# FordyceLab/magnify

Measured on AMD Instinct MI355X. Metric: megapixels/sec through flatfield+segment+ROI-reduce; markers/sec, higher is better.
Workload: dtype u16

## Files before the change

include/magnify_hip.h:

```cpp
#ifndef MAGNIFY_HIP_H
#define MAGNIFY_HIP_H

#include <stddef.h>
#include <stdint.h>

#ifdef __cplusplus
extern "C" {
#endif

#define MG_OK 0
#define MG_EINVAL (-1)
#define MG_ELAUNCH (-2)
#define MG_EIO (-3)

#define MG_U8 0
#define MG_U16 1
#define MG_F32 2
#define MG_F64 3

#define MG_NO_EDGE 100.0f
#define MG_SCORE_SKIPPED (-2.0f)

#define MG_WALK_MAX_Y 65535
#define MG_ZERO_WALK 1024
// ... 74 lines not shown
#define MG_PLANE_MINMAX_WALK 1024
int mg_plane_minmax(const void* d_src, int dtype, int n_planes, int64_t plane_stride, int h, int w,
                    int64_t row_stride, double* d_minmax, void* stream);


#define MG_ROTATE_WALK 2048
int mg_affine_bilinear(const void* d_src, void* d_dst, int dtype, int64_t n_planes, int h, int w,
                       const double* matrix, const double* offset, double* d_minmax, void* stream);

int64_t mg_shading_workspace_bytes(int n, int w);
int64_t mg_shading_offset(int n, int w, int field);
int mg_shading_downsample(const void* d_tiles, int dtype, int64_t n, int ty, int tx, int w, float* d_out, void* stream);
int mg_shading_prepare(void* d_ws, int n, int w, void* stream);
int mg_shading_dct2(void* d_ws, int n, int w, const double* d_in, double* d_out, int inverse, void* stream);
int mg_shading_alm_begin(void* d_ws, int n, int w, int get_darkfield, int max_iterations, double mu, double lam_f,
                         double lam_d, double tol, double norm_f, double b_up, void* stream);
int mg_shading_alm_iterate(void* d_ws, int n, int w, int k, int get_darkfield, void* stream);
int mg_shading_reweight(void* d_ws, int n, int w, double epsilon, void* stream);
int mg_shading_upsample(const double* d_flat_w, const double* d_dark_w, int w, int ty, int tx, double* d_partial,
                        float* d_flat, float* d_dark, void* stream);
#define MG_SHADING_APPLY_WALK 2048
#define MG_SHADING_SETUP_WALK 1024
int mg_shading_apply_stitch(const void* d_tiles, int dtype, int n_fields, int64_t planes_per_field, int n_tile_rows,
                            int n_tile_cols, int ty, int tx, int overlap, const float* d_flat, const float* d_dark,
                            void* d_image, double* d_minmax, void* stream);
int mg_shading_apply_stitch_blend(const void* d_tiles, int dtype, int n_fields, int64_t planes_per_field,
                                  int n_tile_rows, int n_tile_cols, int ty, int tx, int overlap, const float* d_flat,
                                  const float* d_dark, void* d_image, double* d_minmax, void* stream);

int mg_shading_apply_stitch_shift(const void* d_tiles, int dtype, int n_fields, int64_t planes_per_field,
                                  int n_tile_rows, int n_tile_cols, int ty, int tx, int overlap, const float* d_flat,
                                  const float* d_dark, void* d_image, double* d_minmax, const int32_t* d_shift,
                                  int n_tables, int n_time, int blend, void* stream);


int mg_to_uint8_blur(const void* d_src, int dtype, int n_planes, int64_t plane_stride, int h, int w,
                     int64_t row_stride, const double* d_minmax, uint8_t* d_blur, uint8_t* d_u8, void* stream);

int mg_scharr_hist(const uint8_t* d_blur, int n_planes, int h, int w, int mode, const uint32_t* d_base,
                   uint32_t* d_hist, uint32_t* d_scratch, int64_t scratch_words, void* stream);
int64_t mg_scharr_hist_scratch_words(int n_planes, int h, int w, int mode);

int mg_to_uint8_blur_hist(const void* d_src, int dtype, int n_planes, int64_t plane_stride, int h, int w,
                          int64_t row_stride, const double* d_minmax, uint8_t* d_blur, uint8_t* d_u8, uint32_t* d_hist,
                          uint32_t* d_scratch, int64_t scratch_words, void* stream);
int64_t mg_blur_hist_scratch_words(int n_planes, int h, int w);

int mg_edge_thresholds(const uint32_t* d_hist, int n_planes, const int64_t* ranks4, float gamma_low, float gamma_high,
                       int32_t* d_thresh, float* d_quantiles, int32_t* d_unresolved, int32_t* d_state,
                       uint32_t* d_win_base, void* stream);
int mg_edge_thresholds_window(const uint32_t* d_hist_win, int n_planes, int pass, float gamma_low, float gamma_high,
                              int32_t* d_state, uint32_t* d_win_base, int32_t* d_thresh, float* d_quantiles,
                              int32_t* d_unresolved, void* stream);


int mg_canny_nms(const uint8_t* d_blur, int n_planes, int h, int w, const int32_t* d_thresh, uint32_t* d_weak,
                 uint32_t* d_strong, uint32_t* d_class, int64_t words_per_plane, void* stream);
int mg_canny_nms_strips(int w, int* strip_w, int* wave_rows, int* group_rows);

int mg_canny_hysteresis(const uint32_t* d_weak, uint32_t* d_strong, int64_t words_per_plane, int n_planes, int h,
                        int w, uint32_t* d_changed, const uint8_t* d_flags_in, uint8_t* d_flags_out, void* stream);
int mg_hysteresis_tiles(int h, int w, int* tiles_x, int* tiles_y);

#define MG_UNPACK_BITS_WALK 4096
int mg_unpack_bits(const uint32_t* d_bits, int64_t words_per_plane, int n_planes, int64_t n_bits, uint8_t* d_out,
                   void* stream);

int64_t mg_edge_grid_scan_words(int n_planes, int h, int w, int grid);
int mg_edge_grid(const uint32_t* d_edge_bits, int64_t words_per_plane, int n_planes, int h, int w, int grid,
                 int32_t* d_cell_counts, int32_t* d_cell_starts, int32_t* d_num_edges, int32_t* d_coords,
                 int64_t coord_cap, uint64_t* d_scan_state, int32_t* d_edge_totals, int phases, void* stream);

#define MG_EDGE_ANGLES_WALK 1048576
int mg_edge_angles(const uint8_t* d_blur, int n_planes, int h, int w, const int32_t* d_coords, int64_t coord_cap,
                   const int32_t* d_num_edges, float* d_angle, void* stream);


int mg_dedup_layout(int h, int w, int min_r, int max_r, int* n_tile_rows, int* n_tile_cols, int64_t* n_layers,
                    int64_t* bitmap_words);

#define MG_CANDIDATES_WALK 2048
#define MG_CANDIDATES_TAB_WALK 1024
#define MG_CANDIDATES_TAB_FILL 1024
int mg_candidate_circles(const int32_t* d_coords, int64_t coord_cap, const int32_t* d_cell_starts,
                         const int32_t* d_cell_counts, const int32_t* d_num_edges, int n_planes, int h, int w,
                         int grid, const uint64_t* d_seeds, int64_t num_iter, int min_r, int max_r,
                         uint32_t* d_bitmap, int64_t bitmap_words, float* d_raw, void* stream);

int mg_candidate_keys(const int32_t* d_coords, int64_t coord_cap, const int32_t* d_cell_starts,
                      const int32_t* d_cell_counts, const int32_t* d_num_edges, int n_planes, int h, int w, int grid,
                      const uint64_t* d_seeds, int64_t num_iter, int min_r, int max_r, uint32_t* d_keys, float* d_raw,
                      void* stream);

int mg_keys_to_circles(const uint32_t* d_keys, int64_t num_iter, const int32_t* d_cell_starts,
                       const int32_t* d_cell_counts, const int32_t* d_num_edges, int n_planes, int h, int w, int grid,
                       int min_r, int max_r, uint32_t* d_unique_keys, int64_t circle_cap, int32_t* d_tile_ranges,
                       int32_t* d_num_circles, int32_t* d_layer_starts, int counters_clear, void* stream);

int mg_bitmap_to_circles(uint32_t* d_bitmap, int64_t bitmap_words, int n_planes, int h, int w, int min_r,
                         int max_r, int32_t* d_layer_offsets, int32_t* d_circles, int64_t circle_cap,
                         int32_t* d_num_circles, void* stream);

#define MG_SCORE_EXACT_WALK 4096
#define MG_SCORE_PREFILTER_WALK 4096
int mg_score_circles(const float* d_angle, const uint32_t* d_edge_bits, const uint32_t* d_class_bits,
                     int64_t words_per_plane, int n_planes, int h, int w, int32_t* d_circles, int64_t circle_cap,
                     const int32_t* d_layer_offsets, const uint32_t* d_unique_keys, const int32_t* d_tile_ranges,
                     int min_r, int max_r, const int32_t* d_per_rc, const double* d_per_expected,
                     const int32_t* d_per_starts, int per_total, float min_roundness, int write_skipped,
                     int dedup_centres, float* d_scores, int32_t* d_alive, int32_t* d_num_alive, int32_t* d_max_rc,
                     int32_t* d_num_scored, void* stream);

int mg_score_keyed_supported(int min_r, int max_r);
int mg_score_pair_table(uint64_t* out_entries, int cap);
int mg_score_pairs(int r, int32_t* out_rc, int cap);
int mg_score_walk_reads(int r);
int mg_score_circles_keyed(const uint8_t* d_blur, const float* d_angle, const uint32_t* d_edge_bits,
                           const uint32_t* d_class_bits, int64_t words_per_plane, int n_planes, int h, int w,
                           int32_t* d_circles, int64_t circle_cap, const uint32_t* d_unique_keys,
                           const int32_t* d_layer_starts, int min_r, int max_r, const int32_t* d_per_rc,
                           const double* d_per_expected, const int32_t* d_per_starts, int per_total,
                           const uint64_t* d_pair_table, float min_roundness, int write_skipped, float* d_scores,
                           int32_t* d_alive, int32_t* d_num_alive, int32_t* d_max_rc, int32_t* d_num_scored,
                           int32_t* d_surv_list, int64_t surv_cap, int32_t* d_num_surv, int counters_clear,
                           void* stream);

int mg_nms_rounds(const int32_t* d_circles, int64_t circle_cap, const float* d_scores, const int32_t* d_alive,
                  const int32_t* d_num_alive, const int32_t* d_max_rc, int n_planes, int min_dist,
                  const int32_t* d_ring_rc, int ring_len, uint64_t* d_grid, int64_t grid_cap, uint8_t* d_state,
                  int32_t* d_undecided, int64_t undecided_stride, int n_rounds, int counters_clear,
                  const uint32_t* d_tie_keys, int64_t max_alive, const int32_t* d_skip, void* stream);

int mg_nms_same_centre(const int32_t* d_circles, int64_t circle_cap, const float* d_scores, const int32_t* d_alive,
                       const int32_t* d_num_alive, const int32_t* d_max_rc, int n_planes, int min_dist, uint64_t* d_grid,
                       int64_t grid_cap, uint8_t* d_state, const uint32_t* d_tie_keys, int64_t max_alive,
                       const int32_t* d_skip, void* stream);

int mg_nms_cleanup(const int32_t* d_circles, int64_t circle_cap, const float* d_scores, const int32_t* d_alive,
                   const int32_t* d_num_alive, const int32_t* d_max_rc, int n_planes, int min_dist,
                   const int32_t* d_ring_rc, int ring_len, uint64_t* d_grid, int64_t grid_cap, uint8_t* d_state,
                   int64_t max_alive, const int32_t* d_skip, void* stream);

int mg_nms_sparse(const int32_t* d_circles, int64_t circle_cap, const float* d_scores, const int32_t* d_alive,
                  const int32_t* d_num_alive, const int32_t* d_max_rc, int n_planes, int min_dist, const uint32_t* d_dbits,
                  uint8_t* d_state, const uint32_t* d_tie_keys, int32_t* d_done, void* stream);
int mg_nms_sparse_max_dist(void);

#define MG_COLLECT_WALK 8192
int mg_collect_circles(const int32_t* d_circles, int64_t circle_cap, const float* d_scores, const int32_t* d_alive,
                       const int32_t* d_num_alive, const uint8_t* d_state, int keep_all, int n_planes,
                       int32_t* d_out, float* d_out_scores, int64_t out_cap, int32_t* d_num_out,
                       int32_t* d_scratch, const uint32_t* d_tie_keys, int counters_clear, void* stream);


int mg_circle_labels(const int32_t* d_beads, int64_t bead_cap, const int32_t* d_num_beads, int n_planes, int h,
                     int w, const int32_t* d_halfwidths, int max_r, int32_t* d_labels, void* stream);

int mg_roi_gather_reduce_batched(const void* d_image, int dtype, int64_t assay_stride, int n_c, int n_t, int h, int w,
                                 const int32_t* d_beads, const int32_t* d_marker_assay,
                                 const int32_t* d_marker_local, int m, int roi_len, const int32_t* d_labels,
                                 void* d_roi, uint8_t* d_fg, uint8_t* d_bg, double* d_sums, int32_t* d_counts,
                                 void* stream);

int mg_counts_to_offsets(const int32_t* d_counts, int n, int cap, int32_t* d_offsets, void* stream);

#define MG_MARKER_TABLE_WALK 2048
// ... 186 lines not shown
```

magnify_amd/csrc/mg_circles.hip:

```cpp
#include <math.h>
#include <stdlib.h>

#include "mg_common.h"

namespace {

constexpr int NT = 256;

constexpr uint64_t GOLDEN = 0x9E3779B97F4A7C15ull;
__device__ __forceinline__ uint64_t mix64(uint64_t z) {
  z ^= z >> 30;
  z *= 0xBF58476D1CE4E5B9ull;
  z ^= z >> 27;
  z *= 0x94D049BB133111EBull;
  return z ^ (z >> 31);
}
__device__ __forceinline__ uint32_t mix_top32(uint64_t z) { return (uint32_t)(mix64(z) >> 32); }

__device__ __forceinline__ uint32_t div_f64(double x, double d, double inv_d) {
  uint32_t q = (uint32_t)(x * inv_d);
  const double r = fma(-(double)q, d, x);
  if (r < 0.0) --q;
  else if (r >= d) ++q;
  return q;
}

__device__ __forceinline__ uint64_t div_u64(uint64_t n, uint64_t d, double inv_d) {
  uint64_t q = (uint64_t)((double)n * inv_d);
  int64_t r = (int64_t)(n - q * d);
  if (r < 0) {
    --q;
    r += (int64_t)d;
  }
  if (r >= (int64_t)d) ++q;
  return q;
}

constexpr double BISECTOR_EPS = (double)1e-20f;
__device__ __forceinline__ double2 bisector(int d_row, int d_col) {
  const double m = (double)(-d_col) / ((double)d_row + BISECTOR_EPS);
  return make_double2(m, 0.5 * (double)d_row - m * (0.5 * (double)d_col));
}

struct DivFull {
  __device__ __forceinline__ double operator()(double num, double den) const { return num / den; }
};
struct DivUnscaled {
  __device__ __forceinline__ double operator()(double num, double den) const {
    if (!(fabs(den) > 0.0 && fabs(den) < 1.0e300)) return num / den;
    double y = __builtin_amdgcn_rcp(den);
    double e = fma(-den, y, 1.0);
    y = fma(y, e, y);
    e = fma(-den, y, 1.0);
    y = fma(y, e, y);
    double q = num * y;
    const double r = fma(-den, q, num);
    return fma(r, y, q);
  }
};

template <class Div>
__device__ __forceinline__ float3 circle_from_bisectors(double2 l1, double2 l2, int p0r, int p0c, Div div) {
  const float c_col = (float)div(l1.y - l2.y, l2.x - l1.x + BISECTOR_EPS);
  const float c_row = (float)(l1.x * (double)c_col + l1.y);
  const float rad = sqrtf(c_row * c_row + c_col * c_col);
  return make_float3((float)((double)c_row + (double)p0r), (float)((double)c_col + (double)p0c), rad);
}

__device__ __forceinline__ void store_raw(float* __restrict__ d_raw, int64_t index, float3 c) {
  if (!d_raw) return;
  float* o = d_raw + index * 3;
  o[0] = c.x;
  o[1] = c.y;
  o[2] = c.z;
}

template <class Emit>
__device__ __forceinline__ void candidate_cell(float3 c, int h, int w, int min_r, int max_r, int ntc, Emit&& emit) {
  if (!(c.z >= (float)min_r && c.z <= (float)max_r)) return;
  const float rr = rintf(c.x), rc = rintf(c.y);
  if (!(fabsf(rr) < 1.0e9f && fabsf(rc) < 1.0e9f)) return;
  const int ir = (int)rr, ic = (int)rc, irad = (int)rintf(c.z);
  if (ir + irad < 0 || ic + irad < 0 || ir - irad >= h || ic - irad >= w) return;
  const int pr = ir + max_r, pc = ic + max_r;
  emit((pr >> 6) * ntc + (pc >> 6), irad - min_r, pr & 63, pc & 63);
}

template <bool FAST>
__global__ __launch_bounds__(NT) void k_candidates(const int32_t* __restrict__ d_coords, int64_t coord_cap,
                                                   const int32_t* __restrict__ d_starts,
                                                   const int32_t* __restrict__ d_counts,
                                                   const int32_t* __restrict__ d_num_edges, int h, int w, int grid,
                                                   int gc, int n_cells, const uint64_t* __restrict__ d_seeds,
                                                   int64_t num_iter, int min_r, int max_r,
                                                   uint32_t* __restrict__ d_bitmap, int64_t bitmap_words,
                                                   float* __restrict__ d_raw, uint32_t* __restrict__ d_keys) {
  const int plane = blockIdx.y;
  const uint32_t n_edges = (uint32_t)d_num_edges[plane];
  if (n_edges == 0) return;
  const int32_t* coords = d_coords + (int64_t)plane * coord_cap * 2;
  const int32_t* starts = d_starts + (int64_t)plane * n_cells;
  const int32_t* counts = d_counts + (int64_t)plane * n_cells;
  const uint64_t seed = d_seeds[plane];
  const int ntc = (w + 2 * max_r + 63) >> 6, nr = max_r - min_r + 1;
  uint32_t* bitmap = d_bitmap ? d_bitmap + (int64_t)plane * bitmap_words : nullptr;
  uint32_t* keys = d_keys ? d_keys + (int64_t)plane * num_iter : nullptr;
  const double inv_iter = 1.0 / (double)num_iter;
  const int64_t it0 = (int64_t)blockIdx.x * NT + threadIdx.x, stride = (int64_t)gridDim.x * NT;
  uint64_t zbase = seed + ((uint64_t)it0 * 3ull + 1ull) * GOLDEN;
  const uint64_t zstep = (uint64_t)stride * 3ull * GOLDEN;
  const uint32_t eq = FAST ? n_edges / (uint32_t)num_iter : 0u;
  const double er = FAST ? (double)(n_edges - eq * (uint32_t)num_iter) : 0.0, dk = (double)num_iter;
  const uint32_t gmagic = grid > 1 ? 0xFFFFFFFFu / (uint32_t)grid + 1u : 0u;
  for (int64_t it = it0; it < num_iter; it += stride, zbase += zstep) {
    uint64_t sa, sb;
    if (FAST) {
      const double x = (double)(uint32_t)it * er;
      sa = (uint64_t)((uint32_t)it * eq + div_f64(x, dk, inv_iter));
      sb = (uint64_t)(((uint32_t)it + 1u) * eq + div_f64(x + er, dk, inv_iter));
    } else {
      sa = div_u64((uint64_t)it * n_edges, (uint64_t)num_iter, inv_iter);
      sb = div_u64(((uint64_t)it + 1) * n_edges, (uint64_t)num_iter, inv_iter);
    }
    const uint64_t width = sb > sa ? sb - sa : 1;
    const uint32_t u0 = (uint32_t)(sa + (((uint64_t)mix_top32(zbase) * width) >> 32));
    const int p0r = coords[2 * (int64_t)u0], p0c = coords[2 * (int64_t)u0 + 1];
    const int cell = FAST ? (int)(__umulhi((uint32_t)p0r, gmagic) * (uint32_t)gc + __umulhi((uint32_t)p0c, gmagic))
                           : (p0r / grid) * gc + (p0c / grid);
    const uint32_t cnt = (uint32_t)counts[cell];
    const int64_t base = starts[cell];
    const uint64_t z12 = mix64(zbase + GOLDEN);
    const int64_t i1 = base + (int64_t)__umulhi((uint32_t)(z12 >> 32), cnt);
    const int64_t i2 = base + (int64_t)__umulhi((uint32_t)z12, cnt);
    const double2 l1 = bisector(coords[2 * i1] - p0r, coords[2 * i1 + 1] - p0c);
    const double2 l2 = bisector(coords[2 * i2] - p0r, coords[2 * i2 + 1] - p0c);
    const float3 c = circle_from_bisectors(l1, l2, p0r, p0c, DivFull{});
    store_raw(d_raw, (int64_t)plane * num_iter + it, c);
    uint32_t key = MG_NO_KEY;
    candidate_cell(c, h, w, min_r, max_r, ntc, [&](int tile, int layer, int row, int col) {
      if (keys) {
        key = mg_key_pack(tile, layer, row, col);
      } else {
        const int64_t bit = (((int64_t)tile * nr + layer) << 12) + (row << 6) + col;
        atomicOr(&bitmap[bit >> 5], 1u << (bit & 31));
      }
    });
    if (keys) keys[it] = key;
  }
}

constexpr int CT = 1024;
constexpr int MAX_TAB_GRID = 32;

__global__ __launch_bounds__(CT) void k_candidates_tab(const int32_t* __restrict__ d_coords, int64_t coord_cap,
                                                       const int32_t* __restrict__ d_starts,
                                                       const int32_t* __restrict__ d_counts,
                                                       const int32_t* __restrict__ d_num_edges, int h, int w, int grid,
                                                       int gc, int n_cells, const uint64_t* __restrict__ d_seeds,
                                                       uint32_t num_iter, int min_r, int max_r,
                                                       float* __restrict__ d_raw, uint32_t* __restrict__ d_keys) {
  extern __shared__ double2 s_tab[];
  const int plane = blockIdx.y;
  const uint32_t n_edges = (uint32_t)d_num_edges[plane];
  if (n_edges == 0) return;
  const int g1 = grid - 1, span = 2 * grid - 1;
  for (int i = threadIdx.x; i < span * span; i += CT) s_tab[i] = bisector(i / span - g1, i - (i / span) * span - g1);
  __syncthreads();
  const int32_t* coords = d_coords + (int64_t)plane * coord_cap * 2;
  const int32_t* starts = d_starts + (int64_t)plane * n_cells;
  const int32_t* counts = d_counts + (int64_t)plane * n_cells;
  const uint64_t seed = d_seeds[plane];
  const int ntc = (w + 2 * max_r + 63) >> 6;
  uint32_t* keys = d_keys ? d_keys + (int64_t)plane * num_iter : nullptr;
  const uint32_t K = num_iter;
  const uint32_t it0 = blockIdx.x * CT + threadIdx.x, stride = gridDim.x * CT;
  if (it0 >= K) return;
  const uint32_t eq = n_edges / K, er = n_edges - eq * K;
  const double inv_k = 1.0 / (double)K;
  const uint64_t x0 = (uint64_t)it0 * er;
  const uint64_t q0 = div_u64(x0, K, inv_k);
  uint32_t sa = it0 * eq + (uint32_t)q0, rem = (uint32_t)(x0 - q0 * K);
  const uint64_t xs = (uint64_t)stride * er;
  const uint64_t qs = div_u64(xs, K, inv_k);
  const uint32_t sa_step = stride * eq + (uint32_t)qs, rem_step = (uint32_t)(xs - qs * K);
  uint64_t zbase = seed + ((uint64_t)it0 * 3ull + 1ull) * GOLDEN;
  const uint64_t zstep = (uint64_t)stride * 3ull * GOLDEN;
  const uint32_t gmagic = 0xFFFFFFFFu / (uint32_t)grid + 1u;
  for (uint32_t it = it0; it < K; it += stride, zbase += zstep) {
    const uint32_t sb = sa + eq + (rem + er >= K ? 1u : 0u);
    uint32_t u0 = sa;
    if (sb > sa + 1u) u0 = sa + __umulhi(mix_top32(zbase), sb - sa);
    {
      const uint32_t t = rem + rem_step;
      const bool carry = t >= K;
      sa += sa_step + (carry ? 1u : 0u);
      rem = carry ? t - K : t;
    }
    const int2 p0 = reinterpret_cast<const int2*>(coords)[u0];
    const int p0r = p0.x, p0c = p0.y;
    const int cell = (int)(__umulhi((uint32_t)p0r, gmagic) * (uint32_t)gc + __umulhi((uint32_t)p0c, gmagic));
    const uint32_t cnt = (uint32_t)counts[cell];
    const uint32_t base = (uint32_t)starts[cell];
    const uint64_t z12 = mix64(zbase + GOLDEN);
    const uint32_t i1 = base + __umulhi((uint32_t)(z12 >> 32), cnt);
    const uint32_t i2 = base + __umulhi((uint32_t)z12, cnt);
    const int2 p1 = reinterpret_cast<const int2*>(coords)[i1], p2 = reinterpret_cast<const int2*>(coords)[i2];
    const int d1r = p1.x - p0r, d1c = p1.y - p0c, d2r = p2.x - p0r, d2c = p2.y - p0c;
    double2 l1, l2;
    if ((uint32_t)(d1r + g1) < (uint32_t)span && (uint32_t)(d1c + g1) < (uint32_t)span &&
        (uint32_t)(d2r + g1) < (uint32_t)span && (uint32_t)(d2c + g1) < (uint32_t)span) {
      l1 = s_tab[(d1r + g1) * span + d1c + g1], l2 = s_tab[(d2r + g1) * span + d2c + g1];
    } else {
      l1 = bisector(d1r, d1c), l2 = bisector(d2r, d2c);
    }
    const float3 c = circle_from_bisectors(l1, l2, p0r, p0c, DivUnscaled{});
    store_raw(d_raw, ((int64_t)plane * num_iter + it), c);
    uint32_t key = MG_NO_KEY;
    candidate_cell(c, h, w, min_r, max_r, ntc, [&](int tile, int layer, int row, int col) { key = mg_key_pack(tile, layer, row, col); });
    if (keys) keys[it] = key;
  }
}

constexpr int TS = 64;
constexpr int LAYER_WORDS = 128;

__global__ __launch_bounds__(NT) void k_layer_count(const uint32_t* __restrict__ d_bitmap, int64_t bitmap_words,
                                                    int n_layers, int32_t* __restrict__ d_layer_offsets) {
  const int plane = blockIdx.y;
  const int layer = blockIdx.x * (NT / 64) + (threadIdx.x >> 6);
  if (layer >= n_layers) return;
  const int lane = threadIdx.x & 63;
  const uint2 v = reinterpret_cast<const uint2*>(d_bitmap + (int64_t)plane * bitmap_words +
                                                 (int64_t)layer * LAYER_WORDS)[lane];
  const int c = mg_wave_sum_i32(__popc(v.x) + __popc(v.y));
  if (lane == 0) d_layer_offsets[(int64_t)plane * (n_layers + 1) + layer] = c;
}

constexpr int MAX_RANGES = 64;
constexpr int DEDUP_TX = 2;
struct Keys4 {
  uint32_t k[4];
};

template <int TX>
__global__ __launch_bounds__(NT) void k_tile_dedup(const uint32_t* __restrict__ d_keys, int64_t num_iter,
                                                   const int32_t* __restrict__ d_starts,
                                                   const int32_t* __restrict__ d_counts,
                                                   const int32_t* __restrict__ d_num_edges, int h, int w, int grid,
                                                   int gr, int gc, int ntc, int nr, int max_r,
                                                   uint32_t* __restrict__ d_ukeys, int64_t circle_cap,
                                                   int32_t* __restrict__ d_tile_ranges, int n_tiles,
                                                   int32_t* __restrict__ d_num_circles,
                                                   int32_t* __restrict__ d_layer_starts) {
  extern __shared__ uint32_t lbits[];
  __shared__ long long s_lo[MAX_RANGES];
  __shared__ int s_pre[MAX_RANGES + 1];
  __shared__ int s_cnt[TX * 32 + 1];
  __shared__ int s_base;
  const int lin = blockIdx.x + gridDim.x * (blockIdx.y + gridDim.y * blockIdx.z);
  const int plane = lin % (int)gridDim.z, group = lin / (int)gridDim.z;
  const int tr = group / (int)gridDim.x, tc0 = (group - tr * (int)gridDim.x) * TX;
  const int ntx = min(TX, ntc - tc0);
  const int tile0 = tr * ntc + tc0;
  const int words = nr * LAYER_WORDS;
  for (int i = threadIdx.x; i < ntx * words; i += NT) lbits[i] = 0u;
  const long long n_edges = d_num_edges[plane];
  const int reach = max_r + 2;
  const int y0 = max(tr * TS - max_r - reach, 0), y1 = min(tr * TS + TS - 1 - max_r + reach, h - 1);
  const int x0 = max(tc0 * TS - max_r - reach, 0), x1 = min((tc0 + ntx) * TS - 1 - max_r + reach, w - 1);
  int n_ranges = 0;
  if (n_edges > 0 && y0 <= y1 && x0 <= x1) {
    const int cr0 = y0 / grid, cr1 = y1 / grid, cc0 = x0 / grid, cc1 = x1 / grid;
    n_ranges = cr1 - cr0 + 1;
    if ((int)threadIdx.x < n_ranges) {
      const int32_t* starts = d_starts + (int64_t)plane * gr * gc;
      const int32_t* counts = d_counts + (int64_t)plane * gr * gc;
      const int cr = cr0 + threadIdx.x;
      const long long ea = starts[cr * gc + cc0], eb = (long long)starts[cr * gc + cc1] + counts[cr * gc + cc1];
      long long lo = 0, hi = 0;
      if (eb > ea) {
        const double kpe = (double)num_iter / (double)n_edges;
        hi = min((long long)((double)eb * kpe) + 3, (long long)num_iter);
        lo = min(max((long long)((double)ea * kpe) - 2, 0ll), hi);
      }
      s_lo[threadIdx.x] = lo;
      s_pre[threadIdx.x + 1] = (int)(hi - lo);
    }
  }
  __syncthreads();
  if (threadIdx.x == 0) {
    s_pre[0] = 0;
    for (int r = 0; r < n_ranges; ++r) s_pre[r + 1] += s_pre[r];
  }
  __syncthreads();
  const uint32_t* keys = d_keys + (int64_t)plane * num_iter;
  constexpr int KB = 8;
  for (int r = 0; r < n_ranges; ++r) {
    const uint32_t* kr = keys + s_lo[r];
    const int len = s_pre[r + 1] - s_pre[r];
    for (int base = threadIdx.x; base < len; base += NT * KB) {
      uint32_t kv[KB];
#pragma unroll
      for (int u = 0; u < KB; ++u) {
// ... 717 lines not shown
        list[k] = idx;
        list[out_cap + 2 * (int64_t)k] = (int32_t)(uint32_t)key;
        list[out_cap + 2 * (int64_t)k + 1] = (int32_t)(uint32_t)(key >> 32);
      }
    }
  }
}

constexpr int RANK_CHUNK = 2048;

__global__ __launch_bounds__(NT) void k_collect_rank(const int32_t* __restrict__ d_circles, int64_t circle_cap,
                                                     const float* __restrict__ d_scores,
                                                     const int32_t* __restrict__ d_scratch,
                                                     int32_t* __restrict__ d_num_out, int64_t out_cap,
                                                     int32_t* __restrict__ d_out, float* __restrict__ d_out_scores) {
  __shared__ __attribute__((aligned(16))) uint64_t keys[RANK_CHUNK];
  const int plane = blockIdx.y;
  const int m = (int)min((int64_t)d_num_out[plane], out_cap);
  const int32_t* list = d_scratch + (int64_t)plane * 3 * out_cap;
  const uint32_t* kw = reinterpret_cast<const uint32_t*>(list + out_cap);
  const float* scores = d_scores + (int64_t)plane * circle_cap;
  for (int64_t a0 = (int64_t)blockIdx.x * NT; a0 < m; a0 += (int64_t)gridDim.x * NT) {
    const int64_t a = a0 + threadIdx.x;
    const int idx = a < m ? list[a] : 0;
    const uint64_t key = a < m ? (((uint64_t)kw[2 * a + 1] << 32) | kw[2 * a]) : 0;
    int rank = 0;
    for (int c0 = 0; c0 < m; c0 += RANK_CHUNK) {
      const int cn = min(RANK_CHUNK, m - c0);
      __syncthreads();
      for (int b = threadIdx.x; b < cn; b += NT) keys[b] = ((uint64_t)kw[2 * (int64_t)(c0 + b) + 1] << 32) | kw[2 * (int64_t)(c0 + b)];
      __syncthreads();
      const uint4* k4 = reinterpret_cast<const uint4*>(keys);
      int b = 0;
      for (; b + 8 <= cn; b += 8) {
        uint4 q[4];
#pragma unroll
        for (int u = 0; u < 4; ++u) q[u] = k4[(b >> 1) + u];
#pragma unroll
        for (int u = 0; u < 4; ++u) {
          rank += (((uint64_t)q[u].y << 32) | q[u].x) < key;
          rank += (((uint64_t)q[u].w << 32) | q[u].z) < key;
        }
      }
      for (; b < cn; ++b) rank += keys[b] < key;
    }
    if (a < m) {
      const int32_t* c = d_circles + ((int64_t)plane * circle_cap + idx) * 3;
      int32_t* o = d_out + ((int64_t)plane * out_cap + rank) * 3;
      o[0] = c[0];
      o[1] = c[1];
      o[2] = c[2];
      if (d_out_scores) d_out_scores[(int64_t)plane * out_cap + rank] = scores[idx];
    }
  }
}

__global__ void k_clamp_counts(int32_t* d_num_out, int n_planes, int64_t out_cap) {
  const int i = blockIdx.x * blockDim.x + threadIdx.x;
  if (i < n_planes && d_num_out[i] > out_cap) d_num_out[i] = (int32_t)out_cap;
}

inline int grid_x(int64_t n) { return (int)std::max<int64_t>(1, std::min<int64_t>((n + NT - 1) / NT, MG_COLLECT_WALK)); }

}

namespace {
int launch_candidates(const int32_t* d_coords, int64_t coord_cap, const int32_t* d_cell_starts,
                      const int32_t* d_cell_counts, const int32_t* d_num_edges, int n_planes, int h, int w, int grid,
                      const uint64_t* d_seeds, int64_t num_iter, int min_r, int max_r, uint32_t* d_bitmap,
                      int64_t bitmap_words, float* d_raw, uint32_t* d_keys, void* stream) {
  if (!d_coords || !d_cell_starts || !d_cell_counts || !d_num_edges || !d_seeds || (!d_bitmap && !d_keys))
    return MG_EINVAL;
  if (n_planes < 0 || n_planes > 65535 || h <= 0 || w <= 0 || grid <= 0 || num_iter < 0 || min_r < 0 || max_r < min_r)
    return MG_EINVAL;
  if ((double)num_iter * (double)h * (double)w >= 4.0e15) return MG_EINVAL;
  int ntr, ntc, nr;
  int64_t n_layers, need_words;
  if (d_keys && mg_key_layout(h, w, min_r, max_r, &ntr, &ntc, &nr) != MG_OK) return MG_EINVAL;
  if (d_bitmap && (mg_dedup_layout(h, w, min_r, max_r, &ntr, &ntc, &n_layers, &need_words) != MG_OK || bitmap_words < need_words))
    return MG_EINVAL;
  if (n_planes == 0 || num_iter == 0) return MG_OK;
  const int gr = (h + grid - 1) / grid, gc = (w + grid - 1) / grid;
  const bool fast = num_iter < (1ll << 31) && grid > 1 && h <= 65536 && w <= 65536;
  static const bool v1 = getenv("MG_CANDIDATES_V1") != nullptr;
  if (fast && !v1 && d_keys && !d_bitmap && grid <= MAX_TAB_GRID && coord_cap < (1ll << 31)) {
    const int64_t per_plane = (num_iter + CT - 1) / CT;
    int64_t blocks = std::max<int64_t>((num_iter + 32 * CT - 1) / (32 * CT), (MG_CANDIDATES_TAB_FILL + n_planes - 1) / n_planes);
    blocks = std::max<int64_t>(1, std::min<int64_t>(std::min<int64_t>(blocks, per_plane), MG_CANDIDATES_TAB_WALK));
    const int span = 2 * grid - 1;
    static bool tab_attr = false;
    if (!tab_attr) {
      if (hipFuncSetAttribute(reinterpret_cast<const void*>(k_candidates_tab), hipFuncAttributeMaxDynamicSharedMemorySize,
                              (2 * MAX_TAB_GRID - 1) * (2 * MAX_TAB_GRID - 1) * (int)sizeof(double2)) != hipSuccess)
        return MG_ELAUNCH;
      tab_attr = true;
    }
    hipLaunchKernelGGL(k_candidates_tab, dim3((unsigned)blocks, n_planes), dim3(CT), (size_t)span * span * sizeof(double2),
                       mg_stream(stream), d_coords, coord_cap, d_cell_starts, d_cell_counts, d_num_edges, h, w, grid, gc,
                       gr * gc, d_seeds, (uint32_t)num_iter, min_r, max_r, d_raw, d_keys);
    MG_CHECK_LAUNCH();
    return MG_OK;
  }
  hipLaunchKernelGGL(fast ? k_candidates<true> : k_candidates<false>, dim3((unsigned)std::max<int64_t>(1, std::min<int64_t>((num_iter + NT - 1) / NT, MG_CANDIDATES_WALK)), n_planes), dim3(NT), 0,
                     mg_stream(stream), d_coords,
                     coord_cap, d_cell_starts, d_cell_counts, d_num_edges, h, w, grid, gc, gr * gc, d_seeds, num_iter,
                     min_r, max_r, d_bitmap, bitmap_words, d_raw, d_keys);
  MG_CHECK_LAUNCH();
  return MG_OK;
}
}

extern "C" int mg_candidate_circles(const int32_t* d_coords, int64_t coord_cap, const int32_t* d_cell_starts,
                                    const int32_t* d_cell_counts, const int32_t* d_num_edges, int n_planes, int h,
                                    int w, int grid, const uint64_t* d_seeds, int64_t num_iter, int min_r, int max_r,
                                    uint32_t* d_bitmap, int64_t bitmap_words, float* d_raw, void* stream) {
  if (!d_bitmap) return MG_EINVAL;
  return launch_candidates(d_coords, coord_cap, d_cell_starts, d_cell_counts, d_num_edges, n_planes, h, w, grid, d_seeds,
                           num_iter, min_r, max_r, d_bitmap, bitmap_words, d_raw, nullptr, stream);
}

extern "C" int mg_candidate_keys(const int32_t* d_coords, int64_t coord_cap, const int32_t* d_cell_starts,
                                 const int32_t* d_cell_counts, const int32_t* d_num_edges, int n_planes, int h, int w,
                                 int grid, const uint64_t* d_seeds, int64_t num_iter, int min_r, int max_r,
                                 uint32_t* d_keys, float* d_raw, void* stream) {
  if (!d_keys) return MG_EINVAL;
  return launch_candidates(d_coords, coord_cap, d_cell_starts, d_cell_counts, d_num_edges, n_planes, h, w, grid, d_seeds,
                           num_iter, min_r, max_r, nullptr, 0, d_raw, d_keys, stream);
}

extern "C" int mg_dedup_layout(int h, int w, int min_r, int max_r, int* n_tile_rows, int* n_tile_cols,
                               int64_t* n_layers, int64_t* bitmap_words) {
  if (h <= 0 || w <= 0 || min_r < 0 || max_r < min_r || !n_tile_rows || !n_tile_cols || !n_layers || !bitmap_words)
    return MG_EINVAL;
  const int ntr = (h + 2 * max_r + TS - 1) / TS, ntc = (w + 2 * max_r + TS - 1) / TS;
  *n_tile_rows = ntr;
  *n_tile_cols = ntc;
  *n_layers = (int64_t)ntr * ntc * (max_r - min_r + 1);
  *bitmap_words = *n_layers * LAYER_WORDS;
  return MG_OK;
}

extern "C" int mg_bitmap_to_circles(uint32_t* d_bitmap, int64_t bitmap_words, int n_planes, int h, int w, int min_r,
                                    int max_r, int32_t* d_layer_offsets, int32_t* d_circles, int64_t circle_cap,
                                    int32_t* d_num_circles, void* stream) {
  if (!d_bitmap || !d_layer_offsets || !d_circles || !d_num_circles || n_planes < 0 || n_planes > 65535 ||
      circle_cap < 0)
    return MG_EINVAL;
  int ntr, ntc;
  int64_t n_layers, need_words;
  if (mg_dedup_layout(h, w, min_r, max_r, &ntr, &ntc, &n_layers, &need_words) != MG_OK) return MG_EINVAL;
  if (bitmap_words < need_words || n_layers > 0x7FFFFFF0) return MG_EINVAL;
  if (n_planes == 0) return MG_OK;
  const int nl = (int)n_layers, nr = max_r - min_r + 1;
  hipStream_t s = mg_stream(stream);
  const dim3 g((nl + 3) / 4, n_planes);
  hipLaunchKernelGGL(k_layer_count, g, dim3(NT), 0, s, d_bitmap, bitmap_words, nl, d_layer_offsets);
  MG_CHECK_LAUNCH();
  hipLaunchKernelGGL(k_layer_scan, dim3(n_planes), dim3(1024), 0, s, d_layer_offsets, nl, d_num_circles, circle_cap);
  MG_CHECK_LAUNCH();
  hipLaunchKernelGGL(k_layer_emit, g, dim3(NT), 0, s, d_bitmap, bitmap_words, nl, d_layer_offsets, ntc, nr, min_r, max_r,
                     d_circles, circle_cap);
  MG_CHECK_LAUNCH();
  return MG_OK;
}

extern "C" int mg_keys_to_circles(const uint32_t* d_keys, int64_t num_iter, const int32_t* d_cell_starts,
                                  const int32_t* d_cell_counts, const int32_t* d_num_edges, int n_planes, int h, int w,
                                  int grid, int min_r, int max_r, uint32_t* d_unique_keys, int64_t circle_cap,
                                  int32_t* d_tile_ranges, int32_t* d_num_circles, int32_t* d_layer_starts,
                                  int counters_clear, void* stream) {
  if (!d_keys || !d_cell_starts || !d_cell_counts || !d_num_edges || !d_unique_keys || !d_tile_ranges ||
      !d_num_circles || n_planes < 0 || n_planes > 65535 || circle_cap < 0 || num_iter < 0 || grid <= 0)
    return MG_EINVAL;
  int ntr, ntc, nr;
  if (mg_key_layout(h, w, min_r, max_r, &ntr, &ntc, &nr) != MG_OK) return MG_EINVAL;
  if ((TS + 2 * (max_r + 2)) / grid + 2 > MAX_RANGES || num_iter >= (1ll << 31)) return MG_EINVAL;
  if (n_planes == 0) return MG_OK;
  const int gr = (h + grid - 1) / grid, gc = (w + grid - 1) / grid;
  hipStream_t s = mg_stream(stream);
  if (ntr > 65535) return MG_EINVAL;
  if (!counters_clear && mg_zero_async(d_num_circles, (size_t)n_planes * sizeof(int32_t), s) != hipSuccess) return MG_ELAUNCH;
  const int tx = DEDUP_TX;
// ... 195 lines not shown
```

Measured before the change: 227,500.

## Batch candidate-circle iterations per thread and use radius threshold table

The tabulated candidate kernel now handles a run of four consecutive iterations per thread. It gathers all point and cell loads before doing the arithmetic, which lets memory latency overlap, and it writes the keys as one vector store. Radius layer selection compares the squared radius against a host-precomputed threshold table instead of doing an exact sqrt and round, and it uses f32 coordinate adds when raw output is off. Smaller changes include a bit-test guard in the division, mad24 indexing and byte-offset addressing. The risks are more register pressure at 1024 threads per block and narrower eligibility limits on coord_cap.

```diff
diff --git a/include/magnify_hip.h b/include/magnify_hip.h
--- a/include/magnify_hip.h
+++ b/include/magnify_hip.h
@@ -180,6 +180,7 @@
 #define MG_CANDIDATES_WALK 2048
 #define MG_CANDIDATES_TAB_WALK 1024
 #define MG_CANDIDATES_TAB_FILL 1024
+#define MG_CANDIDATES_TAB_RUN 4
 int mg_candidate_circles(const int32_t* d_coords, int64_t coord_cap, const int32_t* d_cell_starts,
                          const int32_t* d_cell_counts, const int32_t* d_num_edges, int n_planes, int h, int w,
                          int grid, const uint64_t* d_seeds, int64_t num_iter, int min_r, int max_r,
diff --git a/magnify_amd/csrc/mg_circles.hip b/magnify_amd/csrc/mg_circles.hip
--- a/magnify_amd/csrc/mg_circles.hip
+++ b/magnify_amd/csrc/mg_circles.hip
@@ -1,7 +1,10 @@
 #include <math.h>
 #include <stdlib.h>
 
+#include <mutex>
+
 #include "mg_common.h"
+#include "mg_radius.h"
 
 namespace {
 
@@ -47,7 +50,7 @@
 };
 struct DivUnscaled {
   __device__ __forceinline__ double operator()(double num, double den) const {
-    if (!(fabs(den) > 0.0 && fabs(den) < 1.0e300)) return num / den;
+    if ((((uint32_t)__double2hiint(den) & 0x7FFFFFFFu) - 0x00100000u) >= 0x7E200000u) return num / den;
     double y = __builtin_amdgcn_rcp(den);
     double e = fma(-den, y, 1.0);
     y = fma(y, e, y);
@@ -60,11 +63,16 @@
 };
 
 template <class Div>
+__device__ __forceinline__ float2 centre_from_bisectors(double2 l1, double2 l2, Div div) {
+  const float c_col = (float)div(l1.y - l2.y, l2.x - l1.x + BISECTOR_EPS);
+  return make_float2((float)(l1.x * (double)c_col + l1.y), c_col);
+}
+__device__ __forceinline__ float image_coord(float c, int p0) { return (float)((double)c + (double)p0); }
+__device__ __forceinline__ float image_coord_f32(float c, int p0) { return c + (float)p0; }
+template <class Div>
 __device__ __forceinline__ float3 circle_from_bisectors(double2 l1, double2 l2, int p0r, int p0c, Div div) {
-  const float c_col = (float)div(l1.y - l2.y, l2.x - l1.x + BISECTOR_EPS);
-  const float c_row = (float)(l1.x * (double)c_col + l1.y);
-  const float rad = sqrtf(c_row * c_row + c_col * c_col);
-  return make_float3((float)((double)c_row + (double)p0r), (float)((double)c_col + (double)p0c), rad);
+  const float2 c = centre_from_bisectors(l1, l2, div);
+  return make_float3(image_coord(c.x, p0r), image_coord(c.y, p0c), sqrtf(c.x * c.x + c.y * c.y));
 }
 
 __device__ __forceinline__ void store_raw(float* __restrict__ d_raw, int64_t index, float3 c) {
@@ -84,6 +92,22 @@
   if (ir + irad < 0 || ic + irad < 0 || ir - irad >= h || ic - irad >= w) return;
   const int pr = ir + max_r, pc = ic + max_r;
   emit((pr >> 6) * ntc + (pc >> 6), irad - min_r, pr & 63, pc & 63);
+}
+
+__device__ __forceinline__ uint32_t mad24(uint32_t a, uint32_t b, uint32_t c) {
+  uint32_t d;
+  asm("v_mad_u32_u24 %0, %1, %2, %3" : "=v"(d) : "v"(a), "s"(b), "v"(c));
+  return d;
+}
+
+__device__ __forceinline__ uint32_t candidate_key(float row, float col, float s, float guess, const MgRadiusTable& rt,
+                                                  const float* t, int h, int w, int ntc) {
+  int layer;
+  const bool in_range = mg_radius_decide(s, guess, rt.lo, rt.hi, t, rt.min_r, rt.max_r, &layer);
+  const float rr = rintf(row), rc = rintf(col), fr = (float)(rt.min_r + layer);
+  if (!(in_range && rr >= -fr && rc >= -fr && rr < (float)h + fr && rc < (float)w + fr)) return MG_NO_KEY;
+  const uint32_t pr = (uint32_t)((int)rr + rt.max_r), pc = (uint32_t)((int)rc + rt.max_r);
+  return mg_key_pack((int)mad24(pr >> 6, (uint32_t)ntc, pc >> 6), layer, (int)(pr & 63u), (int)(pc & 63u));
 }
 
 template <bool FAST>
@@ -151,74 +175,112 @@
 
 constexpr int CT = 1024;
 constexpr int MAX_TAB_GRID = 32;
-
-__global__ __launch_bounds__(CT) void k_candidates_tab(const int32_t* __restrict__ d_coords, int64_t coord_cap,
+template <int RUN>
+struct KeyRun {
+  uint32_t k[RUN];
+};
+
+template <int RUN, bool RAW>
+__global__ __launch_bounds__(CT) void k_candidates_tab(const int32_t* __restrict__ d_coords, uint32_t coord_cap,
                                                        const int32_t* __restrict__ d_starts,
                                                        const int32_t* __restrict__ d_counts,
                                                        const int32_t* __restrict__ d_num_edges, int h, int w, int grid,
                                                        int gc, int n_cells, const uint64_t* __restrict__ d_seeds,
-                                                       uint32_t num_iter, int min_r, int max_r,
+                                                       uint32_t num_iter, MgRadiusTable rt,
                                                        float* __restrict__ d_raw, uint32_t* __restrict__ d_keys) {
   extern __shared__ double2 s_tab[];
+  __shared__ float s_t[MG_RADIUS_MAX_LAYERS + 1];
   const int plane = blockIdx.y;
   const uint32_t n_edges = (uint32_t)d_num_edges[plane];
   if (n_edges == 0) return;
   const int g1 = grid - 1, span = 2 * grid - 1;
   for (int i = threadIdx.x; i < span * span; i += CT) s_tab[i] = bisector(i / span - g1, i - (i / span) * span - g1);
+  if (threadIdx.x <= MG_RADIUS_MAX_LAYERS) s_t[threadIdx.x] = rt.t[threadIdx.x];
   __syncthreads();
-  const int32_t* coords = d_coords + (int64_t)plane * coord_cap * 2;
-  const int32_t* starts = d_starts + (int64_t)plane * n_cells;
-  const int32_t* counts = d_counts + (int64_t)plane * n_cells;
+  const char* coords = reinterpret_cast<const char*>(d_coords + (int64_t)plane * coord_cap * 2);
+  const char* starts = reinterpret_cast<const char*>(d_starts + (int64_t)plane * n_cells);
+  const char* counts = reinterpret_cast<const char*>(d_counts + (int64_t)plane * n_cells);
+  auto point = [&](uint32_t i) { return *reinterpret_cast<const int2*>(coords + (i << 3)); };
   const uint64_t seed = d_seeds[plane];
-  const int ntc = (w + 2 * max_r + 63) >> 6;
-  uint32_t* keys = d_keys ? d_keys + (int64_t)plane * num_iter : nullptr;
+  const int ntc = (w + 2 * rt.max_r + 63) >> 6;
+  uint32_t* keys = d_keys + (int64_t)plane * num_iter;
   const uint32_t K = num_iter;
-  const uint32_t it0 = blockIdx.x * CT + threadIdx.x, stride = gridDim.x * CT;
+  const uint32_t it0 = (blockIdx.x * CT + threadIdx.x) * RUN, stride = gridDim.x * CT * RUN;
   if (it0 >= K) return;
   const uint32_t eq = n_edges / K, er = n_edges - eq * K;
   const double inv_k = 1.0 / (double)K;
   const uint64_t x0 = (uint64_t)it0 * er;
   const uint64_t q0 = div_u64(x0, K, inv_k);
   uint32_t sa = it0 * eq + (uint32_t)q0, rem = (uint32_t)(x0 - q0 * K);
-  const uint64_t xs = (uint64_t)stride * er;
+  const uint64_t xs = (uint64_t)(stride - RUN) * er;
   const uint64_t qs = div_u64(xs, K, inv_k);
-  const uint32_t sa_step = stride * eq + (uint32_t)qs, rem_step = (uint32_t)(xs - qs * K);
+  const uint32_t sa_step = (stride - RUN) * eq + (uint32_t)qs, rem_step = (uint32_t)(xs - qs * K);
   uint64_t zbase = seed + ((uint64_t)it0 * 3ull + 1ull) * GOLDEN;
   const uint64_t zstep = (uint64_t)stride * 3ull * GOLDEN;
   const uint32_t gmagic = 0xFFFFFFFFu / (uint32_t)grid + 1u;
-  for (uint32_t it = it0; it < K; it += stride, zbase += zstep) {
-    const uint32_t sb = sa + eq + (rem + er >= K ? 1u : 0u);
-    uint32_t u0 = sa;
-    if (sb > sa + 1u) u0 = sa + __umulhi(mix_top32(zbase), sb - sa);
+  auto next_stratum = [&]() -> uint32_t {
+    const uint32_t t = rem + er;
+    rem = min(t, t - K);
+    return sa = sa + eq + (t >= K ? 1u : 0u);
+  };
+  auto candidate = [&](uint32_t it, int2 p0, int2 p1, int2 p2) -> uint32_t {
+    const int o_r = p0.x - g1, o_c = p0.y - g1;
+    const uint32_t j1r = (uint32_t)(p1.x - o_r), j1c = (uint32_t)(p1.y - o_c);
+    const uint32_t j2r = (uint32_t)(p2.x - o_r), j2c = (uint32_t)(p2.y - o_c);
+    double2 l1, l2;
+    if (max(max(j1r, j1c), max(j2r, j2c)) < (uint32_t)span) {
+      l1 = s_tab[mad24(j1r, (uint32_t)span, j1c)], l2 = s_tab[mad24(j2r, (uint32_t)span, j2c)];
+    } else {
+      l1 = bisector((int)j1r - g1, (int)j1c - g1), l2 = bisector((int)j2r - g1, (int)j2c - g1);
+    }
+    const float2 c = centre_from_bisectors(l1, l2, DivUnscaled{});
+    const float s = c.x * c.x + c.y * c.y;
+    if (RAW) {
+      const float3 raw = make_float3(image_coord(c.x, p0.x), image_coord(c.y, p0.y), sqrtf(s));
+      store_raw(d_raw, (int64_t)plane * num_iter + it, raw);
+      return candidate_key(raw.x, raw.y, s, raw.z, rt, s_t, h, w, ntc);
+    }
+    return candidate_key(image_coord_f32(c.x, p0.x), image_coord_f32(c.y, p0.y), s, __builtin_amdgcn_sqrtf(s), rt, s_t, h, w, ntc);
+  };
+  auto run_of = [&](auto n, uint32_t it, uint32_t* out) {
+    constexpr int N = decltype(n)::value;
+    int2 p0[N], p1[N], p2[N];
+    uint32_t cell[N];
+    uint32_t a = sa;
+#pragma unroll
+    for (int j = 0; j < N; ++j) {
+      const uint32_t b = next_stratum();
+      uint32_t u0 = a;
+      if (b > a + 1u) u0 = a + __umulhi(mix_top32(zbase + (uint64_t)(3 * j) * GOLDEN), b - a);
+      p0[j] = point(u0);
+      a = b;
+    }
+#pragma unroll
+    for (int j = 0; j < N; ++j)
+      cell[j] = (__umul24(__umulhi((uint32_t)p0[j].x, gmagic), (uint32_t)gc) + __umulhi((uint32_t)p0[j].y, gmagic)) << 2;
+#pragma unroll
+    for (int j = 0; j < N; ++j) {
+      const uint32_t cnt = *reinterpret_cast<const uint32_t*>(counts + cell[j]);
+      const uint32_t base = *reinterpret_cast<const uint32_t*>(starts + cell[j]);
+      const uint64_t z12 = mix64(zbase + (uint64_t)(3 * j + 1) * GOLDEN);
+      p1[j] = point(base + __umulhi((uint32_t)(z12 >> 32), cnt)), p2[j] = point(base + __umulhi((uint32_t)z12, cnt));
+    }
+#pragma unroll
+    for (int j = 0; j < N; ++j) out[j] = candidate(it + j, p0[j], p1[j], p2[j]);
+  };
+  uint32_t it = it0;
+  for (; it + RUN <= K; it += stride, zbase += zstep) {
+    KeyRun<RUN> run;
+    run_of(std::integral_constant<int, RUN>{}, it, run.k);
+    *reinterpret_cast<KeyRun<RUN>*>(keys + it) = run;
     {
       const uint32_t t = rem + rem_step;
       const bool carry = t >= K;
       sa += sa_step + (carry ? 1u : 0u);
       rem = carry ? t - K : t;
     }
-    const int2 p0 = reinterpret_cast<const int2*>(coords)[u0];
-    const int p0r = p0.x, p0c = p0.y;
-    const int cell = (int)(__umulhi((uint32_t)p0r, gmagic) * (uint32_t)gc + __umulhi((uint32_t)p0c, gmagic));
-    const uint32_t cnt = (uint32_t)counts[cell];
-    const uint32_t base = (uint32_t)starts[cell];
-    const uint64_t z12 = mix64(zbase + GOLDEN);
-    const uint32_t i1 = base + __umulhi((uint32_t)(z12 >> 32), cnt);
-    const uint32_t i2 = base + __umulhi((uint32_t)z12, cnt);
-    const int2 p1 = reinterpret_cast<const int2*>(coords)[i1], p2 = reinterpret_cast<const int2*>(coords)[i2];
-    const int d1r = p1.x - p0r, d1c = p1.y - p0c, d2r = p2.x - p0r, d2c = p2.y - p0c;
-    double2 l1, l2;
-    if ((uint32_t)(d1r + g1) < (uint32_t)span && (uint32_t)(d1c + g1) < (uint32_t)span &&
-        (uint32_t)(d2r + g1) < (uint32_t)span && (uint32_t)(d2c + g1) < (uint32_t)span) {
-      l1 = s_tab[(d1r + g1) * span + d1c + g1], l2 = s_tab[(d2r + g1) * span + d2c + g1];
-    } else {
-      l1 = bisector(d1r, d1c), l2 = bisector(d2r, d2c);
-    }
-    const float3 c = circle_from_bisectors(l1, l2, p0r, p0c, DivUnscaled{});
-    store_raw(d_raw, ((int64_t)plane * num_iter + it), c);
-    uint32_t key = MG_NO_KEY;
-    candidate_cell(c, h, w, min_r, max_r, ntc, [&](int tile, int layer, int row, int col) { key = mg_key_pack(tile, layer, row, col); });
-    if (keys) keys[it] = key;
-  }
+  }
+  for (; it < K; ++it, zbase += 3ull * GOLDEN) run_of(std::integral_constant<int, 1>{}, it, keys + it);
 }
 
 constexpr int TS = 64;
@@ -1102,22 +1164,34 @@
   if (n_planes == 0 || num_iter == 0) return MG_OK;
   const int gr = (h + grid - 1) / grid, gc = (w + grid - 1) / grid;
   const bool fast = num_iter < (1ll << 31) && grid > 1 && h <= 65536 && w <= 65536;
-  static const bool v1 = getenv("MG_CANDIDATES_V1") != nullptr;
-  if (fast && !v1 && d_keys && !d_bitmap && grid <= MAX_TAB_GRID && coord_cap < (1ll << 31)) {
-    const int64_t per_plane = (num_iter + CT - 1) / CT;
+  const bool v1 = getenv("MG_CANDIDATES_V1") != nullptr;
+  if (fast && !v1 && d_keys && !d_bitmap && grid <= MAX_TAB_GRID && coord_cap < (1ll << 29) && (int64_t)gr * gc < (1ll << 30)) {
+    constexpr int RUN = MG_CANDIDATES_TAB_RUN;
+    int64_t walk = MG_CANDIDATES_TAB_WALK;
+    if (const char* e = getenv("MG_CANDIDATES_TAB_WALK")) walk = std::max<int64_t>(1, std::min<int64_t>(walk, atoll(e)));
+    const int64_t per_plane = (num_iter + CT * RUN - 1) / (CT * RUN);
     int64_t blocks = std::max<int64_t>((num_iter + 32 * CT - 1) / (32 * CT), (MG_CANDIDATES_TAB_FILL + n_planes - 1) / n_planes);
-    blocks = std::max<int64_t>(1, std::min<int64_t>(std::min<int64_t>(blocks, per_plane), MG_CANDIDATES_TAB_WALK));
+    blocks = std::max<int64_t>(1, std::min<int64_t>(std::min<int64_t>(blocks, per_plane), walk));
     const int span = 2 * grid - 1;
-    static bool tab_attr = false;
-    if (!tab_attr) {
-      if (hipFuncSetAttribute(reinterpret_cast<const void*>(k_candidates_tab), hipFuncAttributeMaxDynamicSharedMemorySize,
-                              (2 * MAX_TAB_GRID - 1) * (2 * MAX_TAB_GRID - 1) * (int)sizeof(double2)) != hipSuccess)
-        return MG_ELAUNCH;
-      tab_attr = true;
-    }
-    hipLaunchKernelGGL(k_candidates_tab, dim3((unsigned)blocks, n_planes), dim3(CT), (size_t)span * span * sizeof(double2),
-                       mg_stream(stream), d_coords, coord_cap, d_cell_starts, d_cell_counts, d_num_edges, h, w, grid, gc,
-                       gr * gc, d_seeds, (uint32_t)num_iter, min_r, max_r, d_raw, d_keys);
+    const auto k_candidates_tab_run = d_raw ? k_candidates_tab<RUN, true> : k_candidates_tab<RUN, false>;
+    static std::mutex mu;
+    static bool tab_attr[2] = {false, false};
+    static MgRadiusTable rt = {0.0f, 0.0f, {}, -1, -1};
+    MgRadiusTable table;
+    {
+      std::lock_guard<std::mutex> lock(mu);
+      if (!tab_attr[d_raw != nullptr]) {
+        if (hipFuncSetAttribute(reinterpret_cast<const void*>(k_candidates_tab_run), hipFuncAttributeMaxDynamicSharedMemorySize,
+                                (2 * MAX_TAB_GRID - 1) * (2 * MAX_TAB_GRID - 1) * (int)sizeof(double2)) != hipSuccess)
+          return MG_ELAUNCH;
+        tab_attr[d_raw != nullptr] = true;
+      }
+      if (rt.min_r != min_r || rt.max_r != max_r) mg_radius_table(min_r, max_r, &rt);
+      table = rt;
+    }
+    hipLaunchKernelGGL(k_candidates_tab_run, dim3((unsigned)blocks, n_planes), dim3(CT), (size_t)span * span * sizeof(double2),
+                       mg_stream(stream), d_coords, (uint32_t)coord_cap, d_cell_starts, d_cell_counts, d_num_edges, h, w, grid, gc,
+                       gr * gc, d_seeds, (uint32_t)num_iter, table, d_raw, d_keys);
     MG_CHECK_LAUNCH();
     return MG_OK;
   }
diff --git a/magnify_amd/csrc/mg_radius.h b/magnify_amd/csrc/mg_radius.h
--- /dev/null
+++ b/magnify_amd/csrc/mg_radius.h
@@ -0,0 +1,71 @@
+#pragma once
+#include <math.h>
+#include <stdint.h>
+#include <string.h>
+
+#if defined(__HIPCC__)
+#define MG_RADIUS_HD __host__ __device__ inline
+#else
+#define MG_RADIUS_HD inline
+#endif
+
+constexpr int MG_RADIUS_MAX_LAYERS = 32;
+
+struct MgRadiusTable {
+  float lo, hi;
+  float t[MG_RADIUS_MAX_LAYERS + 1];
+  int min_r, max_r;
+};
+
+MG_RADIUS_HD bool mg_radius_decide(float s, float guess, float lo, float hi, const float* t, int min_r, int max_r,
+                                   int* layer) {
+#if defined(__HIP_DEVICE_COMPILE__)
+  const float g = __builtin_amdgcn_fmed3f(rintf(guess), (float)min_r, (float)max_r);
+#else
+  const float g = fminf(fmaxf(rintf(guess), (float)min_r), (float)max_r);
+#endif
+  const int i = (int)g - min_r;
+  *layer = i - (s < t[i] ? 1 : 0) + (s >= t[i + 1] ? 1 : 0);
+  return s >= lo && s <= hi;
+}
+MG_RADIUS_HD int mg_radius_layer(float s, float guess, float lo, float hi, const float* t, int min_r, int max_r) {
+  int layer;
+  return mg_radius_decide(s, guess, lo, hi, t, min_r, max_r, &layer) ? layer : -1;
+}
+
+inline float mg_radius_from_bits(uint32_t b) {
+  float f;
+  memcpy(&f, &b, sizeof f);
+  return f;
+}
+
+template <class Pred>
+inline float mg_radius_first(Pred pred) {
+  uint32_t lo = 0u, hi = 0x7F800000u;
+  while (lo < hi) {
+    const uint32_t mid = lo + (hi - lo) / 2u;
+    if (pred(mg_radius_from_bits(mid))) hi = mid;
+    else lo = mid + 1u;
+  }
+  return mg_radius_from_bits(lo);
+}
+
+inline void mg_radius_table(int min_r, int max_r, MgRadiusTable* tab) {
+  auto root = [](float s) -> float {
+    volatile float v = s;
+    volatile float r = sqrtf(v);
+    return r;
+  };
+  tab->min_r = min_r;
+  tab->max_r = max_r;
+  const float fmin = (float)min_r, fmax = (float)max_r;
+  tab->lo = mg_radius_first([&](float s) { return root(s) >= fmin; });
+  const float above = mg_radius_first([&](float s) { return root(s) > fmax; });
+  uint32_t b;
+  memcpy(&b, &above, sizeof b);
+  tab->hi = mg_radius_from_bits(b - 1u);
+  for (int i = 0; i <= MG_RADIUS_MAX_LAYERS; ++i) {
+    const float k = (float)(min_r + i);
+    tab->t[i] = i <= max_r - min_r + 1 ? mg_radius_first([&](float s) { return rintf(root(s)) >= k; }) : INFINITY;
+  }
+}
```

Result: faster. 234,000, median of 6 (+2.9%).
